# jrl-umi3218/lexls

Measured on AMD Instinct MI355X. Metric: batched fp64 l-QR factorizations/s (factorize+solve), higher is better.
Workload: dtype f64

## Files before the change

lexls_amd/csrc/lqr_qtol_body.inc:

```
            static_assert(NS >= 1 && NS <= 4 && MD <= 16 && (MD % 4) == 0, "shape limits of the row layout / two row parts of even size");
            constexpr int NH  = 2;
            constexpr int RP  = MD / NH;
            constexpr int HP  = RP / 2;
            constexpr int kHandoffStride = 8 * MD + 16;
            constexpr int NIH = NS * HP;
#ifndef LEXLS_QTOL_PF_STEPS
#define LEXLS_QTOL_PF_STEPS 9
#endif
            constexpr int PF_STEPS = LEXLS_QTOL_PF_STEPS < MD ? LEXLS_QTOL_PF_STEPS : MD;
            extern __shared__ double smem[];
            typedef __attribute__((address_space(3))) char lds_char;
            const int lds0 = (int)(unsigned)(size_t)(lds_char *)smem;
            const int lane = threadIdx.x & 63;
            const uint32_t wq = QT_WPB > 1 ? blockIdx.x * QT_WPB + (uint32_t)__builtin_amdgcn_readfirstlane((int)(threadIdx.x >> 6)) : blockIdx.x;
            if (wq * 4u >= a.batch) return;
            if constexpr (EST)
            {
                if (wq == 0 && lane == 0) *count_reset = 0u;
            }
            const int g    = lane >> 4;
            const int gl   = lane & 15;
            const int n    = NV ? NV : (int)a.nVar;
            const int cap  = (int)a.cap;
            const int nObj = (int)a.nObj;
            const uint32_t b  = wq * 4u + (uint32_t)g;
            const uint32_t bb = b < a.batch ? b : a.batch - 1u;
            const bool live   = b < a.batch && !(a.skip && a.skip[bb]);
            const uint32_t pstride = (uint32_t)cap * (uint32_t)(n + 1);
            const double *inw      = a.in + (size_t)wq * 4u * pstride;
            const uint32_t poff    = (bb - wq * 4u) * pstride;
            uint32_t dpack = 0;
            int Frow       = 0;
            if constexpr (RAG)
            {
                static_assert(!EST && MD <= 15 && kQuadMaxObj <= 8, "four bits per level in one word; no estimating ragged form");
                const uint32_t dk = gl < nObj ? a.dims[(size_t)bb * (uint32_t)nObj + (uint32_t)gl] : 0u;
                const int dv      = (int)(dk < (uint32_t)MD ? dk : (uint32_t)MD);
                for_each_index<0, kQuadMaxObj>([&](auto kk) __attribute__((always_inline)) {
                    constexpr int k_ = decltype(kk)::value;
                    dpack |= (uint32_t)gbci<k_>(dv) << (4 * k_);
                });
            }
            auto rag_rows = [&](qt_d2 v, int R, int r, int d, double &lo, double &hi) __attribute__((always_inline)) {
                lo = sel(r < d, sel(R == cap - 1, v.y, v.x), 0.0);
                hi = sel(r + 1 < d, v.y, 0.0);
            };

            double blk0[NS][MD];
#pragma unroll
            for (int s = 0; s < NS; s++)
            {
                const int P       = 16 * s + gl - SIG;
                const int c       = (P >= 0 && P <= n) ? P : 0;
                if constexpr (RAG)
                {
                    const double *colp = inw + (poff + (uint32_t)(c * cap));
                    const int d0       = (int)(dpack & 15u);
#pragma unroll
                    for (int r = 0; r < MD / 2; r++)
                    {
                        const int Rc  = 2 * r < cap - 2 ? 2 * r : cap - 2;
                        const qt_d2 v = *reinterpret_cast<const qt_d2u *>(colp + Rc);
                        rag_rows(v, 2 * r, 2 * r, d0, blk0[s][2 * r], blk0[s][2 * r + 1]);
                    }
                }
                else
                {
                    const qt_d2 *src2 = reinterpret_cast<const qt_d2 *>(inw + (poff + (uint32_t)(c * cap)));
#pragma unroll
                    for (int r = 0; r < MD / 2; r++)
                    {
                        const qt_d2 v      = src2[r];
                        blk0[s][2 * r]     = v.x;
                        blk0[s][2 * r + 1] = v.y;
                    }
                }
            }

            const int o_img   = lds0 + (int)((QT_WPB > 1 ? (threadIdx.x >> 6) * 4u : 0u) + (uint32_t)g) * (int)group_bytes;
            const int o_xs    = o_img + 8 * (int)img_doubles;
            const int o_ex    = o_xs + 8 * 16 * NS;
            const int o_phys  = o_ex + 8 * MD;
            const int o_perm  = o_phys + 64;
            const int o_meta  = o_perm + 64;
            const int o_emap  = o_meta + 16 * kQuadMaxObj;
            const int o_stage = o_emap + 8 * 16 * NS;
            auto D   = [&](int off) -> __attribute__((address_space(3))) double & { return *(__attribute__((address_space(3))) double *)(size_t)(unsigned)off; };
            auto D2  = [&](int off) -> __attribute__((address_space(3))) qt_d2 & { return *(__attribute__((address_space(3))) qt_d2 *)(size_t)(unsigned)off; };
            auto B8  = [&](int off) -> __attribute__((address_space(3))) uint8_t & { return *(__attribute__((address_space(3))) uint8_t *)(size_t)(unsigned)off; };
            auto U32 = [&](int off) -> __attribute__((address_space(3))) uint32_t & { return *(__attribute__((address_space(3))) uint32_t *)(size_t)(unsigned)off; };
            auto U64 = [&](int off) -> __attribute__((address_space(3))) unsigned long long & { return *(__attribute__((address_space(3))) unsigned long long *)(size_t)(unsigned)off; };
            typedef unsigned qt_u4 __attribute__((ext_vector_type(4)));
            auto U4 = [&](int off) -> __attribute__((address_space(3))) qt_u4 & { return *(__attribute__((address_space(3))) qt_u4 *)(size_t)(unsigned)off; };

#pragma unroll
            for (int s = 0; s < 4; s++) B8(o_phys + 16 * s + gl) = (uint8_t)(16 * s + gl);
#pragma unroll
            for (int s = 0; s < NS; s++)
            {
                D(o_emap + 8 * (16 * s + gl)) = 0.0;
                D(o_xs + 8 * (16 * s + gl))   = 0.0;
            }
            quad_lds_fence();

            if (stagger)
            {
                const unsigned simd = __builtin_amdgcn_s_getreg((4 << 0) | (4 << 6) | ((2 - 1) << 11));
                for (unsigned i = 0; i < simd * stagger; i++) __builtin_amdgcn_s_sleep(8);
            }

            const int CH = (n + 1) * HP;
            static_assert(NH * NIH <= 18, "eighteen piece registers");
            uint32_t pieceoff[NH * NIH];
            for_each_index<0, NH * NIH>([&](auto tt) __attribute__((always_inline)) {
                constexpr int t = decltype(tt)::value, h = t / NIH, i = t % NIH;
                int ch        = 16 * i + gl;
                ch            = ch < CH ? ch : CH - 1;
                const int col = ch / HP, m = ch - col * HP;
                if constexpr (RAG)
                    pieceoff[t] = ((uint32_t)(col * cap) << 2) | (uint32_t)m;
                else
                    pieceoff[t] = 8u * (poff + (uint32_t)(col * cap + h * RP + 2 * m));
            });
            static_assert(HP <= 4, "two bits for the pair index of a ragged piece");
            auto prefetch_piece = [&](auto tt, int Flev) __attribute__((always_inline)) {
                constexpr int t = decltype(tt)::value, i = t % NIH;
                if (16 * i < CH)
                {
                    if constexpr (RAG)
                    {
                        constexpr int h = t / NIH;
                        const int R     = Flev + h * RP + 2 * (int)(pieceoff[t] & 3u);
                        qt_pf_load<t>(inw, 8u * (poff + (pieceoff[t] >> 2) + (uint32_t)(R < cap - 2 ? R : cap - 2)));
                    }
                    else
                        qt_pf_load<t>(inw + Flev, pieceoff[t]);
                }
            };

            int rp[NS];
            int rq[NS];
            unsigned long long em[NS];
            int pos[NS];
            int pc[NS];
#pragma unroll
            for (int s = 0; s < NS; s++)
            {
                rp[s]  = o_xs;
                rq[s]  = 0x0c0c0c00;
                em[s]  = 0ull;
                pos[s] = 0;
                pc[s]  = 0;
            }

            int ColIndex   = 0;
            int TotalRank  = 0;
            int imgoff     = 0;
            bool exh       = false;
            bool have_next = false;
            double est2    = 0.0;
            double rsq[NS];
            STAMP_DECL
            STAMP(0)
#ifdef LEXLS_QTOL_CHAIN
            unsigned long long cacc[7] = {0, 0, 0, 0, 0, 0, 0};
#endif
#ifdef LEXLS_WAVE_STAMPS
            unsigned long long lst_t0 = clock64();
#endif

            constexpr bool PEEL = !(EST && NS == 3 && MD == 12);
            struct qt_level
            {
                bool work;
                int F;
                int dlev;
                int Fc;
                int rank;
                bool prefetch;
            };

            auto level_head = [&](auto l0c, const int k, qt_level &L) __attribute__((always_inline)) {
                constexpr bool L0 = decltype(l0c)::value;
                QT_LMARK("level-top")
                L.work = live && !exh;
                L.F    = RAG ? Frow : k * MD;
                L.dlev = RAG ? (int)((dpack >> (4 * k)) & 15u) : MD;
                if constexpr (RAG) Frow += L.dlev;
                L.Fc   = ColIndex;
                L.rank = 0;
                if (__ballot(L.work) == 0ull)
                {
                    if (gl == 0)
                    {
                        U32(o_meta + 16 * k)      = (uint32_t)L.Fc;
                        U32(o_meta + 16 * k + 4)  = 0u;
                        U32(o_meta + 16 * k + 8)  = (uint32_t)imgoff;
                        U32(o_meta + 16 * k + 12) = (uint32_t)(n + 1 - L.Fc);
                    }
                    return false;
                }
                if constexpr (!L0)
                {
                    if ((PEEL || k > 0) && !have_next)
                        for_each_index<0, NH * NIH>([&](auto tt) __attribute__((always_inline)) { prefetch_piece(tt, L.F); });
                }
                return true;
            };

            auto level_start = [&](const int k, const qt_level &L, double (&blk)[NS][MD]) __attribute__((always_inline)) {
                const int F = L.F, dlev = L.dlev;
                (void)F, (void)dlev;
                QT_MARK("level-start")
#pragma unroll
                for (int s = 0; s < NS; s++)
                {
                    const int P  = 16 * s + gl - SIG;
                    const int ph = (int)B8(o_phys + (P >= 0 && P < n ? P : 0));
                    pc[s]        = (P >= 0 && P < n) ? ph : (P == n ? n : 0);
                    pos[s]       = (P >= 0 && P <= n) ? P : 0x3fffff;
                }
#pragma unroll
                for (int s = 0; s < NS; s++) em[s] = U64(o_emap + 8 * pc[s]);
                if (PEEL || k > 0)
                for_each_index<0, NH>([&](auto hh) __attribute__((always_inline)) {
                    constexpr int h = decltype(hh)::value;
                    QT_MARK1("level-stage", h)
                    if constexpr (h == 0) asm volatile("s_waitcnt vmcnt(0)" ::: "memory");
                    for_each_index<0, NIH>([&](auto ii) __attribute__((always_inline)) {
                        constexpr int i = decltype(ii)::value;
                        if (16 * i < CH)
                        {
                            int ch = 16 * i + gl;
                            ch     = ch < CH ? ch : CH - 1;
                            qt_pf_store_lds<h * NIH + i>(o_stage + 16 * ch);
                        }
                    });
                    quad_lds_fence();
#pragma unroll
                    for (int s = 0; s < NS; s++)
                    {
#pragma unroll
                        for (int m = 0; m < HP; m++)
                        {
                            const qt_d2 v            = D2(o_stage + 16 * (pc[s] * HP + m));
                            if constexpr (RAG)
                                rag_rows(v, F + h * RP + 2 * m, h * RP + 2 * m, dlev, blk[s][h * RP + 2 * m], blk[s][h * RP + 2 * m + 1]);
                            else
                            {
                                blk[s][h * RP + 2 * m]     = v.x;
                                blk[s][h * RP + 2 * m + 1] = v.y;
                            }
                        }
                    }
                    quad_lds_fence();
                });
            };

            auto level_post = [&](auto l0c, const int k, qt_level &L, double (&blk)[NS][MD]) __attribute__((always_inline)) {
                constexpr bool L0 = decltype(l0c)::value;
                const bool work = L.work;
                const int Fc    = L.Fc;
                (void)k;
                STAMP(1)
                LSTAMP(0)
                QT_LMARK("level-post")
                if constexpr (EST)
                {
#pragma unroll
                    for (int s = 0; s < NS; s++)
                    {
                        double t = 0.0;
#pragma unroll
                        for (int r = 0; r < MD; r++) t = dfma(blk[s][r], blk[s][r], t);
                        rsq[s] = t;
                    }
                }
                L.prefetch = (k + 1 < nObj) && (rows_min(work ? Fc : 0x3fffffff) + MD < n);
                have_next  = L.prefetch;
            };

            auto eliminate = [&](const int k, const qt_level &L, double (&blk)[NS][MD]) __attribute__((always_inline)) {
                (void)k;
                const int Fcmax = rows_max(L.work ? L.Fc : 0);
                {
                    auto fetch_u = [&](auto cc, double (&u)[NS]) __attribute__((always_inline)) {
                        constexpr int C  = decltype(cc)::value;
                        constexpr int sc = (C + SIG) / 16, lc = (C + SIG) % 16;
                        const int rowp   = gbci<lc>(rp[sc]);
                        const int selq   = gbci<lc>(rq[sc]);
#pragma unroll
                        for (int s = sc; s < NS; s++)
                        {
                            const unsigned e = __builtin_amdgcn_perm((unsigned)(em[s] >> 32), (unsigned)em[s], (unsigned)selq);
                            u[s]             = D(rowp + (int)(e << 3));
                        }
                    };
                    double ua[NS], ub[NS];
#pragma unroll
                    for (int s = 0; s < NS; s++) ua[s] = ub[s] = 0.0;
                    if (Fcmax > 0) fetch_u(std::integral_constant<int, 0>{}, ua);
                    qt_for_each_while<0, 16 * NS - SIG>(
                        [&](auto cc) __attribute__((always_inline)) { return decltype(cc)::value < Fcmax; },
                        [&](auto cc) __attribute__((always_inline)) {
                            constexpr int C  = decltype(cc)::value;
                            constexpr int sc = (C + SIG) / 16, lc = (C + SIG) % 16;
                            double(&ucur)[NS]  = (C & 1) ? ub : ua;
                            double(&unext)[NS] = (C & 1) ? ua : ub;
                            QT_MARK1("elim", C)
                            if constexpr (NS - sc <= 2)
                            {
                                if constexpr (sc + 1 < NS) qt_gauss_dpp<lc>(blk[sc + 1], blk[sc], ucur[sc + 1]);
                                if constexpr (C + 1 < 16 * NS - SIG)
                                {
                                    if (C + 1 < Fcmax) fetch_u(std::integral_constant<int, C + 1>{}, unext);
                                }
                                qt_gauss_dpp_self<lc>(blk[sc], ucur[sc]);
                            }
                            else
                            {
                                double lr[MD];
                                for_each_index<0, MD>([&](auto rr) {
                                    constexpr int r = decltype(rr)::value;
                                    lr[r]           = gbc<lc>(blk[sc][r]);
                                });
#pragma unroll
                                for (int r = 0; r < MD; r++) blk[sc][r] = dfma(-lr[r], ucur[sc], blk[sc][r]);
                                if constexpr (C + 1 < 16 * NS - SIG)
                                {
                                    if (C + 1 < Fcmax) fetch_u(std::integral_constant<int, C + 1>{}, unext);
                                }
#pragma unroll
                                for (int s = sc + 1; s < NS; s++)
                                {
#pragma unroll
                                    for (int r = 0; r < MD; r++) blk[s][r] = dfma(-lr[r], ucur[s], blk[s][r]);
                                }
                            }
                        });
                    asm volatile("s_nop 1");
                }
                STAMP(7)
                LSTAMP(1)
            };

                auto factor_level = [&](auto l0c, auto s0c, qt_level &L, double (&blk)[NS][MD]) __attribute__((always_inline)) {
                    constexpr bool L0 = decltype(l0c)::value;
                    constexpr int S0 = decltype(s0c)::value;
                    constexpr int SL = NS - S0;
                    static_assert(!L0 || S0 == 0, "level 0 starts at column 0: every slot is live");
                    const bool work = L.work, prefetch = L.prefetch;
                    const int F = L.F, dlev = L.dlev;
                    int &rank = L.rank;
                    QT_LMARK1("hh-pro", S0)
                    double nrm[NS];
#pragma unroll
                    for (int s = S0; s < NS; s++)
                    {
                        double t = 0.0;
#pragma unroll
                        for (int r = 0; r < MD; r++) t = dfma(blk[s][r], blk[s][r], t);
                        nrm[s] = sel(pos[s] >= ColIndex && pos[s] < n, t, qt_with_hi(t, kQtSentinelHi));
                    }
                    bool go = work;
#ifdef LEXLS_QTOL_CHAIN
                    unsigned long long ct[7] = {0, 0, 0, 0, 0, 0, 0}, cp1 = 0;
                    bool cvalid = false;
#endif
                    int cur_lbs = S0, nxt_lbs = S0;
                    bool cur_ispl = false, nxt_ispl = false;
                    unsigned cur_w = 0, nxt_w = 0;
                    double pbest = 0.0;
                    auto decide_local = [&]() __attribute__((always_inline)) {
#pragma unroll
                        for (int s = S0; s < NS; s++)
                        {
                            const int kinv  = (0xFFF - ((s << 4) | gl)) - (pos[s] << 6);
                            const double pv = __hiloint2double(__double2hiint(nrm[s]), (__double2loint(nrm[s]) & ~0xFFF) | kinv);
                            pbest           = s == S0 ? pv : vmax(pbest, pv);
                        }
                        nxt_lbs = ((0xFFF - (__double2loint(pbest) & 0xFFF)) >> 4) & 3;
                    };
                    auto decide_finish = [&](double m) __attribute__((always_inline)) {
                        const int mlo = __double2loint(m);
                        nxt_w         = (unsigned)(0xFFF - (mlo & 0xFFF));
                        nxt_ispl      = ((__double2loint(pbest) ^ mlo) & 0xFFF) == 0;
                    };
                    {
                        decide_local();
                        decide_finish(row_max16(pbest));
                        double colv[MD];
#pragma unroll
                        for (int r = 0; r < MD; r++) colv[r] = blk[S0][r];
#pragma unroll
                        for (int s = S0 + 1; s < NS; s++)
                        {
                            const bool pick = nxt_lbs == s;
#pragma unroll
                            for (int r = 0; r < MD; r++) colv[r] = sel(pick, blk[s][r], colv[r]);
                        }
#pragma unroll
                        for (int r = 0; r < MD; r += 2) D2(o_stage + gl * kHandoffStride + 8 * r) = qt_d2{colv[r], colv[r + 1]};
                        cur_lbs = nxt_lbs, cur_ispl = nxt_ispl, cur_w = nxt_w;
                    }
                    double coln[MD];
                    auto fetch_column = [&](auto jjc, unsigned w) __attribute__((always_inline)) {
                        constexpr int ce0 = decltype(jjc)::value & ~1;
                        quad_lds_fence();
                        const int src = o_stage + (int)(w & 15u) * kHandoffStride;
#pragma unroll
                        for (int r = ce0; r < MD; r += 2)
                        {
                            const qt_d2 v   = D2(src + 8 * r);
                            coln[r]         = v.x;
                            coln[r + 1]     = v.y;
                        }
                    };
                    fetch_column(std::integral_constant<int, 0>{}, cur_w);

                    int pf_issued = 0;
                    qt_for_each_while<0, MD>(
                        [&](auto jc) __attribute__((always_inline)) { return (decltype(jc)::value % 4 != 0) || __ballot(go) != 0ull; },
                        [&](auto cnt) __attribute__((always_inline)) {
                        constexpr int j   = decltype(cnt)::value;
                        constexpr int ce  = j & ~1;
                        constexpr int cen = (j + 1) & ~1;
                        QT_LMARK2("hh-step", S0, j)
                        {
                            constexpr int TOT = NH * NIH, PF_PER = (TOT + PF_STEPS - 1) / PF_STEPS;
                            constexpr int lo = (j * PF_PER < TOT ? j * PF_PER : TOT), hi = ((j + 1) * PF_PER < TOT ? (j + 1) * PF_PER : TOT);
                            if (prefetch) for_each_index<lo, hi>([&](auto tt) __attribute__((always_inline)) { prefetch_piece(tt, F + dlev); });
                            pf_issued = hi;
                        }
                        const bool act = go;
                        CSTAMP(0, (int)cur_w)
                        double col[MD];
#pragma unroll
                        for (int r = ce; r < MD; r++) col[r] = coln[r];
                        FSTAMP(2)
                        CSTAMP(1, __double2loint(col[MD - 1]))
                        CSTAMP_COLLECT
                        const double c0 = col[j];
                        double t0 = 0.0, t1 = 0.0, t2 = 0.0;
#pragma unroll
                        for (int r = j + 1; r < MD; r++)
                        {
                            if ((r - j) % 3 == 1) t0 = dfma(col[r], col[r], t0);
                            if ((r - j) % 3 == 2) t1 = dfma(col[r], col[r], t1);
                            if ((r - j) % 3 == 0) t2 = dfma(col[r], col[r], t2);
                        }
                        const double tailSq = (t0 + t1) + t2;
                        const double fresh  = dfma(c0, c0, tailSq);
                        CSTAMP(2, __double2loint(fresh))
                        const bool cont     = RAG ? (act && !(fresh < a.tol) && j < dlev) : (act && !(fresh < a.tol));
                        go                  = cont;
                        double g, h;
                        {
                            const double y = __builtin_amdgcn_rsq(fresh);
                            g              = fresh * y;
                            h              = 0.5 * y;
                            double r       = dfma(-h, g, 0.5);
                            g              = dfma(g, r, g);
                            h              = dfma(h, r, h);
#ifndef LEXLS_QTOL_ONE_NEWTON
                            r              = dfma(-h, g, 0.5);
                            g              = dfma(g, r, g);
                            h              = dfma(h, r, h);
#endif
                        }
                        const bool neg    = c0 >= 0.0;
                        const double beta = neg ? -g : g;
                        const double ibet = (neg ? -2.0 : 2.0) * h;
                        CSTAMP(3, __double2loint(ibet))
                        const double rden = qt_rcp1(c0 - beta);
                        double dw[NS];
#pragma unroll
                        for (int s = S0; s < NS; s++)
                        {
                            double d0 = 0.0, d1 = 0.0;
#pragma unroll
                            for (int r = j + 1; r < MD; r++)
                            {
                                if ((r - j) & 1)
                                    d0 = dfma(col[r], blk[s][r], d0);
                                else
                                    d1 = dfma(col[r], blk[s][r], d1);
                            }
                            dw[s] = dfma(c0, blk[s][j], d0 + d1);
                        }
                        FSTAMP(3)
                        double gs[NS];
#pragma unroll
                        for (int s = S0; s < NS; s++)
                        {
                            const double t = dw[s] * ibet;
                            gs[s]          = (t - blk[s][j]) * rden;
                            nrm[s]         = dfma(-t, t, nrm[s]);
                            nrm[s]         = sel(cont && cur_ispl && cur_lbs == s, qt_with_hi(nrm[s], kQtSentinelHi), nrm[s]);
                            blk[s][j]      = t * ibet;
                        }
                        CSTAMP(4, __double2hiint(nrm[NS - 1]))
                        const int ppos = (int)(cur_w >> 6);
#pragma unroll
                        for (int s = S0; s < NS; s++)
                        {
                            const bool front = cont && pos[s] == ColIndex;
                            pos[s]           = sel(front, ppos, pos[s]);
                            pos[s]           = sel(cont && cur_ispl && cur_lbs == s, ColIndex, pos[s]);
                        }
                        B8(sel(cont && cur_ispl, o_perm + ColIndex, o_ex + 4 * gl)) = (uint8_t)ppos;
                        if constexpr (EST)
                        {
                            double r2 = rsq[S0];
#pragma unroll
                            for (int s = S0 + 1; s < NS; s++) r2 = sel(cur_lbs == s, rsq[s], r2);
                            est2 = sel(cont && cur_ispl, vmax(est2, r2 * (h * h)), est2);
                        }
                        ColIndex += cont ? 1 : 0;
                        rank += cont ? 1 : 0;
                        const bool full = cont && ColIndex == n;
                        exh             = exh || full;
                        go              = go && !full;
                        FSTAMP(4)
                        if constexpr (j + 1 < MD && SL == 1)
                        {
                            decide_local();
                            double m = pbest;
                            auto upd_rows = [&](auto qq) __attribute__((always_inline)) {
                                constexpr int q = decltype(qq)::value;
#pragma unroll
                                for (int r = j + 1; r < MD; r++)
                                    if ((r - j - 1) % 4 == q) blk[S0][r] = dfma(gs[S0], col[r], blk[S0][r]);
                            };
                            m = dpp_max<0xB1>(m);
                            upd_rows(std::integral_constant<int, 0>{});
                            m = dpp_max<0x4E>(m);
                            upd_rows(std::integral_constant<int, 1>{});
                            m = dpp_max<0x141>(m);
                            upd_rows(std::integral_constant<int, 2>{});
                            m = dpp_max<0x140>(m);
                            upd_rows(std::integral_constant<int, 3>{});
#pragma unroll
                            for (int r = cen; r < MD; r += 2) D2(o_stage + gl * kHandoffStride + 8 * r) = qt_d2{blk[S0][r], blk[S0][r + 1]};
                            decide_finish(m);
                            fetch_column(std::integral_constant<int, j + 1>{}, nxt_w);
                        }
                        else if constexpr (j + 1 < MD)
                        {
                            decide_local();
                            double colv[MD];
                            double gsb = gs[S0];
                            double m   = pbest;
                            auto pick_rows = [&](auto qq) __attribute__((always_inline)) {
                                constexpr int q = decltype(qq)::value;
#pragma unroll
                                for (int r = cen; r < MD; r++)
                                    if ((r - cen) % 4 == q)
                                    {
                                        colv[r] = blk[S0][r];
#pragma unroll
                                        for (int s = S0 + 1; s < NS; s++) colv[r] = sel(nxt_lbs == s, blk[s][r], colv[r]);
                                    }
                            };
                            m = dpp_max<0xB1>(m);
                            pick_rows(std::integral_constant<int, 0>{});
                            m = dpp_max<0x4E>(m);
                            pick_rows(std::integral_constant<int, 1>{});
                            m = dpp_max<0x141>(m);
                            pick_rows(std::integral_constant<int, 2>{});
                            m = dpp_max<0x140>(m);
                            pick_rows(std::integral_constant<int, 3>{});
#pragma unroll
                            for (int s = S0 + 1; s < NS; s++) gsb = sel(nxt_lbs == s, gs[s], gsb);
#pragma unroll
                            for (int r = (cen > j + 1 ? cen : j + 1); r < MD; r++) colv[r] = dfma(gsb, col[r], colv[r]);
#pragma unroll
                            for (int r = cen; r < MD; r += 2) D2(o_stage + gl * kHandoffStride + 8 * r) = qt_d2{colv[r], colv[r + 1]};
                            decide_finish(m);
                            fetch_column(std::integral_constant<int, j + 1>{}, nxt_w);
                        }
                        CSTAMP(5, (int)nxt_w)
                        if constexpr (!(j + 1 < MD && SL == 1))
                        {
#pragma unroll
                            for (int s = S0; s < NS; s++)
                            {
#pragma unroll
                                for (int r = j + 1; r < MD; r++) blk[s][r] = dfma(gs[s], col[r], blk[s][r]);
                            }
                        }
                        cur_lbs = nxt_lbs, cur_ispl = nxt_ispl, cur_w = nxt_w;
                        CSTAMP(6, __double2loint(blk[NS - 1][MD - 1]))
                        FSTAMP(5)
                    });
                    QT_LMARK1("hh-end", S0)
                    if (prefetch)
                        for_each_index<0, NH * NIH>([&](auto tt) __attribute__((always_inline)) {
                            if (decltype(tt)::value >= pf_issued) prefetch_piece(tt, F + dlev);
                        });
                    (void)SL;
                };

            auto level_end = [&](auto l0c, const int k, const qt_level &L, double (&blk)[NS][MD]) __attribute__((always_inline)) {
                constexpr bool L0 = decltype(l0c)::value;
                const bool work = L.work;
                const int Fc = L.Fc, rank = L.rank;
                STAMP(5)
                LSTAMP(2)
                QT_LMARK("level-end")
                const int wk   = n + 1 - Fc;
                const int dump = o_stage + 8 * gl;
                int roff[MD];
#pragma unroll
                for (int p = 0; p < MD; p++) roff[p] = 8 * (p * wk - p * (p + 1) / 2);
#pragma unroll
                for (int s = 0; s < NS; s++)
                {
                    const int P0  = 16 * s + gl - SIG;
                    const bool mv = work && P0 <= n && P0 >= Fc;
                    const int e   = pos[s] - Fc;
                    const int lim = mv ? (e < rank - 1 ? e : rank - 1) : -1;
                    const int base = o_img + 8 * (imgoff + e);
                    if (mv)
                    {
                        QT_LMARK1("level-end-store", s)
#pragma unroll
                        for (int p = 0; p < MD; p++) D(sel(p <= lim, base + roff[p], dump)) = blk[s][p];
                        B8(o_emap + 8 * pc[s] + k) = (uint8_t)e;
                        if (P0 < n) B8(o_phys + pos[s]) = (uint8_t)pc[s];
                    }
                    QT_LMARK1("level-end-maps", s)
                    const bool piv = work && P0 >= Fc && P0 < Fc + rank;
                    const int p    = P0 - Fc;
                    rp[s]          = sel(piv, o_img + 8 * (imgoff + p * wk - p * (p + 1) / 2), rp[s]);
                    rq[s]          = sel(piv, 0x0c0c0c00 | k, rq[s]);
                }
                STAMP(6)
                LSTAMP(3)
                if (gl == 0)
                {
                    U32(o_meta + 16 * k)      = (uint32_t)Fc;
                    U32(o_meta + 16 * k + 4)  = (uint32_t)rank;
                    U32(o_meta + 16 * k + 8)  = (uint32_t)imgoff;
                    U32(o_meta + 16 * k + 12) = (uint32_t)wk;
                }
                quad_lds_fence();
                imgoff += wk * rank - rank * (rank - 1) / 2;
                TotalRank += rank;
            };

            if constexpr (PEEL)
            {
                qt_level L;
                if (level_head(std::true_type{}, 0, L))
                {
#pragma unroll
                    for (int s = 0; s < NS; s++)
                    {
                        const int P = 16 * s + gl - SIG;
                        pc[s]       = (P >= 0 && P <= n) ? P : 0;
                        pos[s]      = (P >= 0 && P <= n) ? P : 0x3fffff;
                        em[s]       = 0ull;
                    }
                    level_post(std::true_type{}, 0, L, blk0);
                    {
                        constexpr int k = 0;
                        (void)k;
                        STAMP(7)
                        LSTAMP(1)
                    }
                    factor_level(std::true_type{}, std::integral_constant<int, 0>{}, L, blk0);
                    level_end(std::true_type{}, 0, L, blk0);
                }
            }

            for (int k = PEEL ? 1 : 0; k < nObj; k++)
            {
                qt_level L;
                if (!level_head(std::false_type{}, k, L)) continue;
                double blk_k[NS][MD];
                double(&blk)[NS][MD] = *(PEEL ? &blk_k : &blk0);
                level_start(k, L, blk);
                level_post(std::false_type{}, k, L, blk);
                eliminate(k, L, blk);
                QT_MARK("hh-select")
                {
                    const int s0 = (rows_min(L.work ? L.Fc : 0x3fffffff) + SIG) >> 4;
                    if (NS > 3 && s0 >= 3)
                        factor_level(std::false_type{}, std::integral_constant<int, (NS > 3 ? 3 : 0)>{}, L, blk);
                    else if (NS > 2 && s0 >= 2)
                        factor_level(std::false_type{}, std::integral_constant<int, (NS > 2 ? 2 : 0)>{}, L, blk);
                    else if (NS > 1 && s0 >= 1)
                        factor_level(std::false_type{}, std::integral_constant<int, (NS > 1 ? 1 : 0)>{}, L, blk);
                    else
                        factor_level(std::false_type{}, std::integral_constant<int, 0>{}, L, blk);
                }
                level_end(std::false_type{}, k, L, blk);
            }

            QT_MARK("solve-top")
            const int o_zero = o_xs + 8 * (16 * NS - 1);
            for (int k = nObj; k--;)
            {
                QT_MARK("solve-level")
                const qt_u4 mt = U4(o_meta + 16 * k);
                const int rank = live ? (int)mt.y : 0;
                const int rmax = rows_max(rank);
                if (rmax == 0) continue;
                const int Fc = (int)mt.x, ok = (int)mt.z, wk = (int)mt.w;
                const int c0   = Fc + rank;
                const int acc  = rank > 0 ? TotalRank - c0 : 0;
                const int amax = rows_max(acc);
                const int p    = gl < rank ? gl : 0;
                const int row  = o_img + 8 * (ok + p * wk - p * (p + 1) / 2);
                double col[MD];
#pragma unroll
                for (int j = 1; j < MD; j++) col[j] = D(sel(j < rank && gl < j, row + 8 * j, o_zero));
                double sv = D(sel(gl < rank, row + 8 * (n - Fc), o_zero));
                for (int base = 0; base < amax; base += 16)
                {
                    QT_MARK("solve-trip")
                    const bool have = base + gl < acc;
                    const int c     = have ? c0 + base + gl : 16 * NS - 1;
                    const int ph    = (int)B8(o_phys + c);
                    const int offv  = have ? (int)B8(o_emap + 8 * ph + k) : 0;
                    const double xv = D(o_xs + 8 * c);
                    double uj[16];
                    for_each_index<0, 16>([&](auto jj) {
                        constexpr int j = decltype(jj)::value;
                        uj[j]           = D(row + 8 * gbci<j>(offv));
                    });
                    __builtin_amdgcn_sched_barrier(0);
                    double s0 = 0.0, s1 = 0.0;
                    for_each_index<0, 16>([&](auto jj) {
                        constexpr int j = decltype(jj)::value;
                        if (j & 1)
                            s1 = dfma(-uj[j], gbc<j>(xv), s1);
                        else
                            s0 = dfma(-uj[j], gbc<j>(xv), s0);
                    });
                    sv += s0 + s1;
                }
                QT_MARK("solve-tail")
                sv = sel(gl < rank, sv, 0.0);
                for_each_index<1, MD>([&](auto jj) {
                    constexpr int j = MD - decltype(jj)::value;
                    sv = dfma(-col[j], gbc<j>(sv), sv);
                });
                D(sel(gl < rank, o_xs + 8 * (Fc + gl), o_stage + 8 * gl)) = sv;
                quad_lds_fence();
            }
            STAMP(9)
            QT_MARK("output")
            if (live)
            {
#pragma unroll
                for (int s = 0; s < NS; s++)
                {
                    const int P = 16 * s + gl;
                    if (P < n)
                    {
                        a.x[(size_t)b * n + B8(o_phys + P)] = D(o_xs + 8 * P);
                        a.perm[(size_t)b * n + P]           = (P < TotalRank) ? (uint32_t)B8(o_perm + P) : (uint32_t)P;
                    }
                }
                if (gl < nObj)
                {
                    a.fcol[(size_t)b * nObj + gl] = U32(o_meta + 16 * gl);
                    a.rank[(size_t)b * nObj + gl] = U32(o_meta + 16 * gl + 4);
                }
                if (gl == 0) a.totalrank[b] = (uint32_t)TotalRank;
            }
            if constexpr (EST)
            {
                const double e2 = row_max16(est2);
                if (gl == 0 && live) est_out[b] = e2 > 0.0 ? 2.0 * qt_sqrt(e2) : 0.0;
            }
            STAMP(10)
            STAMP_WRITE
#ifdef LEXLS_QTOL_CHAIN
            if (lane == 0)
                for (int i_ = 0; i_ < 7; i_++) a.lambda[(size_t)b * (n + cap) + 30 + i_] = (double)cacc[i_];
#endif
```

lexls_amd/csrc/lqr_qtol_impl.h:

```cpp
#pragma once
#include "lqr_quad_impl.h"

#include <cstdlib>


namespace lexls
{
    namespace
    {
        __device__ __forceinline__ double qt_rcp(double x)
        {
            double y = __builtin_amdgcn_rcp(x);
            double e = dfma(-x, y, 1.0);
            y        = dfma(y, e, y);
            e        = dfma(-x, y, 1.0);
            return dfma(y, e, y);
        }

        __device__ __forceinline__ double qt_rcp1(double x)
        {
            const double y = __builtin_amdgcn_rcp(x);
            return dfma(y, dfma(-x, y, 1.0), y);
        }

        __device__ __forceinline__ double qt_sqrt(double x)
        {
            const double y = __builtin_amdgcn_rsq(x);
            double g       = x * y;
            double h       = 0.5 * y;
            const double r = dfma(-h, g, 0.5);
            g              = dfma(g, r, g);
            h              = dfma(h, r, h);
            double d       = dfma(-g, g, x);
            g              = dfma(d, h, g);
            d              = dfma(-g, g, x);
            return dfma(d, h, g);
        }

        __device__ __forceinline__ double qt_with_hi(double v, int hi) { return __hiloint2double(hi, __double2loint(v)); }

#ifdef LEXLS_WAVE_STAMPS_FINE
#define FSTAMP(i) if constexpr (S0 == LEXLS_WAVE_STAMPS_FINE) STAMP(i)
#else
#define FSTAMP(i)
#endif
#ifdef LEXLS_QTOL_CHAIN
#define CSTAMP(i, val)                                                                                     \
    if constexpr (S0 == LEXLS_QTOL_CHAIN)                                                                  \
    {                                                                                                      \
        int dummy_;                                                                                        \
        asm volatile("v_mov_b32 %1, %2\n\ts_memtime %0" : "=s"(ct[i]), "=v"(dummy_) : "v"(val));         \
    }
#define CSTAMP_COLLECT                                                                                     \
    if constexpr (S0 == LEXLS_QTOL_CHAIN)                                                                  \
    {                                                                                                      \
        asm volatile("s_waitcnt lgkmcnt(0)" ::: "memory");                                                 \
        if (cvalid)                                                                                        \
        {                                                                                                  \
            cacc[2] += ct[2] - cp1; cacc[3] += ct[3] - ct[2]; cacc[4] += ct[4] - ct[3];                     \
            cacc[5] += ct[5] - ct[4]; cacc[6] += ct[6] - ct[5]; cacc[0] += ct[0] - ct[6];                   \
        }                                                                                                  \
        cacc[1] += ct[1] - ct[0];                                                                          \
        cp1    = ct[1];                                                                                    \
        cvalid = true;                                                                                     \
    }
#else
#define CSTAMP(i, val)
#define CSTAMP_COLLECT
#endif
#ifdef LEXLS_WAVE_STAMPS
#define LSTAMP(ph)                                                                                   \
    {                                                                                                \
        const unsigned long long t_ = clock64();                                                     \
        if (gl == 0 && live) a.lambda[(size_t)b * (n + cap) + 11 + 4 * k + (ph)] = (double)(t_ - lst_t0); \
        lst_t0 = t_;                                                                                 \
    }
#else
#define LSTAMP(ph)
#endif
#ifdef LEXLS_QTOL_MARKS
#define QT_MARK(name) asm volatile("; qtol-region " name);
#define QT_MARK1(name, i) asm volatile("; qtol-region " name " %0" ::"i"(i));
#define QT_MARK2(name, i, j) asm volatile("; qtol-region " name " %0 %1" ::"n"(i), "n"(j));
#else
#define QT_MARK(name)
#define QT_MARK1(name, i)
#define QT_MARK2(name, i, j)
#endif
#define QT_LMARK(name)        if constexpr (L0) { QT_MARK("level0-" name) } else { QT_MARK(name) }
#define QT_LMARK1(name, i)    if constexpr (L0) { QT_MARK1("level0-" name, i) } else { QT_MARK1(name, i) }
#define QT_LMARK2(name, i, j) if constexpr (L0) { QT_MARK2("level0-" name, i, j) } else { QT_MARK2(name, i, j) }
        template <int B, int E, class P, class F>
        __device__ __forceinline__ void qt_for_each_while(P &&pred, F &&f)
        {
            if constexpr (B < E)
            {
                if (pred(std::integral_constant<int, B>{}))
                {
                    f(std::integral_constant<int, B>{});
                    qt_for_each_while<B + 1, E>(pred, f);
                }
            }
        }

        typedef double qt_d2 __attribute__((ext_vector_type(2)));
        typedef qt_d2 qt_d2u __attribute__((aligned(8)));


#define QT_PF_LIST(X) X(0, 184, 187) X(1, 188, 191) X(2, 192, 195) X(3, 196, 199) X(4, 200, 203) X(5, 204, 207) X(6, 208, 211) X(7, 212, 215) X(8, 216, 219) \
    X(9, 220, 223) X(10, 224, 227) X(11, 228, 231) X(12, 232, 235) X(13, 236, 239) X(14, 240, 243) X(15, 244, 247) X(16, 248, 251) X(17, 252, 255)
        template <int T>
        __device__ __forceinline__ void qt_pf_load(const double *base, uint32_t byte_offset)
        {
#define QT_PF_LOAD(t, lo, hi) \
    if constexpr (T == t) asm volatile("global_load_dwordx4 a[" #lo ":" #hi "], %0, %1" ::"v"(byte_offset), "s"(base) : "memory", "a" #lo, "a" #hi);
            QT_PF_LIST(QT_PF_LOAD)
#undef QT_PF_LOAD
        }
        template <int T>
        __device__ __forceinline__ void qt_pf_store_lds(int lds_byte_address)
        {
#define QT_PF_STORE(t, lo, hi) \
    if constexpr (T == t) asm volatile("ds_write_b128 %0, a[" #lo ":" #hi "]" ::"v"(lds_byte_address) : "memory");
            QT_PF_LIST(QT_PF_STORE)
#undef QT_PF_STORE
        }

#define QT_FD(i) "v_fmac_f64_dpp %[d" #i "], %[s" #i "], -%[u] row_newbcast:%[l] row_mask:0xf bank_mask:0xf\n\t"
#define QT_FS(i) "v_fmac_f64_dpp %[d" #i "], %[d" #i "], -%[u] row_newbcast:%[l] row_mask:0xf bank_mask:0xf\n\t"
#define QT_FO(i) [d##i] "+v"(d[i])
#define QT_FI(i) [s##i] "v"(s[i])
        template <int L, int MD>
        __device__ __forceinline__ void qt_gauss_dpp(double (&d)[MD], const double (&s)[MD], double u)
        {
            static_assert(MD == 8 || MD == 12, "operand lists below");
            if constexpr (MD == 8)
                asm volatile("s_nop 1\n\t" QT_FD(0) QT_FD(1) QT_FD(2) QT_FD(3) QT_FD(4) QT_FD(5) QT_FD(6) QT_FD(7)
                             : QT_FO(0), QT_FO(1), QT_FO(2), QT_FO(3), QT_FO(4), QT_FO(5), QT_FO(6), QT_FO(7)
                             : QT_FI(0), QT_FI(1), QT_FI(2), QT_FI(3), QT_FI(4), QT_FI(5), QT_FI(6), QT_FI(7), [u] "v"(u), [l] "n"(L));
            else
                asm volatile("s_nop 1\n\t" QT_FD(0) QT_FD(1) QT_FD(2) QT_FD(3) QT_FD(4) QT_FD(5) QT_FD(6) QT_FD(7) QT_FD(8) QT_FD(9) QT_FD(10) QT_FD(11)
                             : QT_FO(0), QT_FO(1), QT_FO(2), QT_FO(3), QT_FO(4), QT_FO(5), QT_FO(6), QT_FO(7), QT_FO(8), QT_FO(9), QT_FO(10), QT_FO(11)
                             : QT_FI(0), QT_FI(1), QT_FI(2), QT_FI(3), QT_FI(4), QT_FI(5), QT_FI(6), QT_FI(7), QT_FI(8), QT_FI(9), QT_FI(10), QT_FI(11),
                               [u] "v"(u), [l] "n"(L));
        }
        template <int L, int MD>
        __device__ __forceinline__ void qt_gauss_dpp_self(double (&d)[MD], double u)
        {
            static_assert(MD == 8 || MD == 12, "operand lists below");
            if constexpr (MD == 8)
                asm volatile("s_nop 1\n\t" QT_FS(0) QT_FS(1) QT_FS(2) QT_FS(3) QT_FS(4) QT_FS(5) QT_FS(6) QT_FS(7)
                             : QT_FO(0), QT_FO(1), QT_FO(2), QT_FO(3), QT_FO(4), QT_FO(5), QT_FO(6), QT_FO(7)
                             : [u] "v"(u), [l] "n"(L));
            else
                asm volatile("s_nop 1\n\t" QT_FS(0) QT_FS(1) QT_FS(2) QT_FS(3) QT_FS(4) QT_FS(5) QT_FS(6) QT_FS(7) QT_FS(8) QT_FS(9) QT_FS(10) QT_FS(11)
                             : QT_FO(0), QT_FO(1), QT_FO(2), QT_FO(3), QT_FO(4), QT_FO(5), QT_FO(6), QT_FO(7), QT_FO(8), QT_FO(9), QT_FO(10), QT_FO(11)
                             : [u] "v"(u), [l] "n"(L));
        }
#undef QT_FD
#undef QT_FS
#undef QT_FO
#undef QT_FI

        constexpr int kQtSentinelHi = (int)0xFFE00000;

        template <int NS, int MD, int SIG, int NV>
        __global__ __launch_bounds__(64 * QT_WPB) void lqr_qtol_kernel(LseArgs a, uint32_t img_doubles, uint32_t group_bytes, uint32_t stagger)
        {
            constexpr bool EST           = false;
            constexpr bool RAG           = false;
            double *const est_out        = nullptr;
            uint32_t *const count_reset  = nullptr;
#include "lqr_qtol_body.inc"
        }

        template <int NS, int MD, int SIG, int NV>
        __global__ __launch_bounds__(64 * QT_WPB) void lqr_qtol_rag_kernel(LseArgs a, uint32_t img_doubles, uint32_t group_bytes, uint32_t stagger)
        {
            constexpr bool EST           = false;
            constexpr bool RAG           = true;
            double *const est_out        = nullptr;
            uint32_t *const count_reset  = nullptr;
#include "lqr_qtol_body.inc"
        }

        template <int NS, int MD, int SIG, int NV>
        __global__ __launch_bounds__(64 * QT_WPB) void lqr_qtol_est_kernel(LseArgs a, uint32_t img_doubles, uint32_t group_bytes, uint32_t stagger, double *est_out,
                                                                          uint32_t *count_reset)
        {
            constexpr bool EST = true;
            constexpr bool RAG = false;
            if constexpr (NS == 3 && MD == 12 && NV == 0)
            {
#include "lqr_qtol_body_unpeeled.inc"
            }
            else
            {
#include "lqr_qtol_body.inc"
            }
        }

        template <int NS, int MD, int SIG, int NV, bool EST = false, bool RAG = false>
        hipError_t launch_qtol_t(const LseArgs &a, hipStream_t s, double *est_out = nullptr, uint32_t *count_reset = nullptr)
        {
            static_assert(!(EST && RAG), "no estimating ragged form");
            const void *kfn;
            if constexpr (RAG)
                kfn = reinterpret_cast<const void *>(lqr_qtol_rag_kernel<NS, MD, SIG, NV>);
            else if constexpr (EST)
                kfn = reinterpret_cast<const void *>(lqr_qtol_est_kernel<NS, MD, SIG, NV>);
            else
                kfn = reinterpret_cast<const void *>(lqr_qtol_kernel<NS, MD, SIG, NV>);
            const uint32_t img  = qtol_image_doubles(a.nVar, a.nObj, MD);
            const size_t gbytes = qtol_group_bytes<NS, MD>(a.nVar, a.nObj);
            const size_t lds    = qtol_lds_bytes<NS, MD>(a.nVar, a.nObj);
            if (lds > kMaxLdsBytes || a.nObj > (uint32_t)kQuadMaxObj || a.nVar + 1 + SIG > 16u * NS || a.nVar > 63u || (NV && a.nVar != (uint32_t)NV)) return hipErrorInvalidValue;
            if ((reinterpret_cast<uintptr_t>(a.in) & (RAG ? 7u : 15u)) || a.nfixed || a.reg_type != 0) return hipErrorInvalidValue;
            if (RAG ? (a.cap < 2u || !a.dims) : (a.uniform_dim != (uint32_t)MD || (a.cap & 1u))) return hipErrorInvalidValue;
            if (lds > 64 * 1024)
            {
                static size_t granted[64] = {0};
                int dev = 0;
                if (hipGetDevice(&dev) != hipSuccess || dev < 0 || dev >= 64) dev = -1;
                if (dev < 0 || granted[dev] < lds)
                {
                    hipError_t e = hipFuncSetAttribute(kfn, hipFuncAttributeMaxDynamicSharedMemorySize, (int)lds);
                    if (e != hipSuccess) return e;
                    if (dev >= 0) granted[dev] = lds;
                }
            }
            const uint32_t blocks = (a.batch + 4u * QT_WPB - 1u) / (4u * QT_WPB);
            static const uint32_t stagger = std::getenv("LEXLS_QTOL_STAGGER") ? (uint32_t)std::atoi(std::getenv("LEXLS_QTOL_STAGGER")) : 0u;
            if constexpr (RAG)
                hipLaunchKernelGGL((lqr_qtol_rag_kernel<NS, MD, SIG, NV>), dim3(blocks), dim3(64 * QT_WPB), lds, s, a, img, (uint32_t)gbytes, stagger);
            else if constexpr (EST)
                hipLaunchKernelGGL((lqr_qtol_est_kernel<NS, MD, SIG, NV>), dim3(blocks), dim3(64 * QT_WPB), lds, s, a, img, (uint32_t)gbytes, stagger, est_out, count_reset);
            else
                hipLaunchKernelGGL((lqr_qtol_kernel<NS, MD, SIG, NV>), dim3(blocks), dim3(64 * QT_WPB), lds, s, a, img, (uint32_t)gbytes, stagger);
            return hipGetLastError();
        }
    }
}

#define LEXLS_QTOL_INSTANCE(NAME, NS, MD, SIG, NV) \
    namespace lexls { hipError_t NAME(const LseArgs &a, hipStream_t s) { return launch_qtol_t<NS, MD, SIG, NV>(a, s); } }
#define LEXLS_QTOL_INSTANCE_EST(NAME, NS, MD, SIG, NV) \
    namespace lexls { hipError_t NAME(const LseArgs &a, hipStream_t s, double *est_out, uint32_t *count_reset) { return launch_qtol_t<NS, MD, SIG, NV, true>(a, s, est_out, count_reset); } }
#define LEXLS_QTOL_INSTANCE_RAG(NAME, NS, MD, SIG, NV) \
    namespace lexls { hipError_t NAME(const LseArgs &a, hipStream_t s) { return launch_qtol_t<NS, MD, SIG, NV, false, true>(a, s); } }
```

Measured before the change: 103.7 million.

## Retire the lone leading column slot after step zero in the factor level

Adds a specialised factor_level form used when every row's level starts on the last column of slot NS-2. After Householder step 0 that slot's remaining column is written out to the image and moved into the last slot through LDS. Later steps then loop over one fewer slot, cutting the FMA, norm and select work. The cost is an extra LDS exchange and fence, a larger code footprint and more register pressure. The path only runs for compile-time shapes where qt_retire_reachable holds and the runtime uniformity test passes.

```diff
diff --git a/lexls_amd/csrc/lqr_qtol_body.inc b/lexls_amd/csrc/lqr_qtol_body.inc
--- a/lexls_amd/csrc/lqr_qtol_body.inc
+++ b/lexls_amd/csrc/lqr_qtol_body.inc
@@ -170,6 +170,8 @@
 #endif
 
             constexpr bool PEEL = !(EST && NS == 3 && MD == 12);
+            constexpr int kRetireSlot = NS - 2;
+            constexpr bool RETIRE     = !EST && !RAG && PEEL && NV > 0 && qt_retire_reachable(NS, MD, SIG, NV) && 8 * (NV + 1) * RP >= 17 * kHandoffStride;
             struct qt_level
             {
                 bool work;
@@ -344,15 +346,18 @@
                 LSTAMP(1)
             };
 
-                auto factor_level = [&](auto l0c, auto s0c, qt_level &L, double (&blk)[NS][MD]) __attribute__((always_inline)) {
+                auto factor_level = [&](auto l0c, auto s0c, auto retc, const int k, qt_level &L, double (&blk)[NS][MD]) __attribute__((always_inline)) {
                     constexpr bool L0 = decltype(l0c)::value;
                     constexpr int S0 = decltype(s0c)::value;
+                    constexpr bool RET = decltype(retc)::value;
                     constexpr int SL = NS - S0;
                     static_assert(!L0 || S0 == 0, "level 0 starts at column 0: every slot is live");
+                    static_assert(!RET || (RETIRE && !L0 && S0 == kRetireSlot && SL == 2), "the retiring form: two live slots, one behind step 0");
+                    (void)k;
                     const bool work = L.work, prefetch = L.prefetch;
                     const int F = L.F, dlev = L.dlev;
                     int &rank = L.rank;
-                    QT_LMARK1("hh-pro", S0)
+                    if constexpr (RET) { QT_MARK1("hh-ret-pro", S0) } else { QT_LMARK1("hh-pro", S0) }
                     double nrm[NS];
 #pragma unroll
                     for (int s = S0; s < NS; s++)
@@ -371,13 +376,14 @@
                     bool cur_ispl = false, nxt_ispl = false;
                     unsigned cur_w = 0, nxt_w = 0;
                     double pbest = 0.0;
-                    auto decide_local = [&]() __attribute__((always_inline)) {
-#pragma unroll
-                        for (int s = S0; s < NS; s++)
+                    auto decide_local = [&](auto loc) __attribute__((always_inline)) {
+                        constexpr int LO = decltype(loc)::value;
+#pragma unroll
+                        for (int s = LO; s < NS; s++)
                         {
                             const int kinv  = (0xFFF - ((s << 4) | gl)) - (pos[s] << 6);
                             const double pv = __hiloint2double(__double2hiint(nrm[s]), (__double2loint(nrm[s]) & ~0xFFF) | kinv);
-                            pbest           = s == S0 ? pv : vmax(pbest, pv);
+                            pbest           = s == LO ? pv : vmax(pbest, pv);
                         }
                         nxt_lbs = ((0xFFF - (__double2loint(pbest) & 0xFFF)) >> 4) & 3;
                     };
@@ -387,7 +393,7 @@
                         nxt_ispl      = ((__double2loint(pbest) ^ mlo) & 0xFFF) == 0;
                     };
                     {
-                        decide_local();
+                        decide_local(std::integral_constant<int, S0>{});
                         decide_finish(row_max16(pbest));
                         double colv[MD];
 #pragma unroll
@@ -425,7 +431,12 @@
                         constexpr int j   = decltype(cnt)::value;
                         constexpr int ce  = j & ~1;
                         constexpr int cen = (j + 1) & ~1;
-                        QT_LMARK2("hh-step", S0, j)
+                        constexpr int SJ  = (RET && j >= 1) ? S0 + 1 : S0;
+                        constexpr int SLJ = NS - SJ;
+                        if constexpr (RET) { QT_MARK2("hh-ret-step", S0, j) } else { QT_LMARK2("hh-step", S0, j) }
+                        const unsigned w0 = cur_w;
+                        const bool ispl0  = cur_ispl;
+                        (void)w0, (void)ispl0;
                         {
                             constexpr int TOT = NH * NIH, PF_PER = (TOT + PF_STEPS - 1) / PF_STEPS;
                             constexpr int lo = (j * PF_PER < TOT ? j * PF_PER : TOT), hi = ((j + 1) * PF_PER < TOT ? (j + 1) * PF_PER : TOT);
@@ -475,7 +486,7 @@
                         const double rden = qt_rcp1(c0 - beta);
                         double dw[NS];
 #pragma unroll
-                        for (int s = S0; s < NS; s++)
+                        for (int s = SJ; s < NS; s++)
                         {
                             double d0 = 0.0, d1 = 0.0;
 #pragma unroll
@@ -491,7 +502,7 @@
                         FSTAMP(3)
                         double gs[NS];
 #pragma unroll
-                        for (int s = S0; s < NS; s++)
+                        for (int s = SJ; s < NS; s++)
                         {
                             const double t = dw[s] * ibet;
                             gs[s]          = (t - blk[s][j]) * rden;
@@ -502,7 +513,7 @@
                         CSTAMP(4, __double2hiint(nrm[NS - 1]))
                         const int ppos = (int)(cur_w >> 6);
 #pragma unroll
-                        for (int s = S0; s < NS; s++)
+                        for (int s = SJ; s < NS; s++)
                         {
                             const bool front = cont && pos[s] == ColIndex;
                             pos[s]           = sel(front, ppos, pos[s]);
@@ -511,9 +522,9 @@
                         B8(sel(cont && cur_ispl, o_perm + ColIndex, o_ex + 4 * gl)) = (uint8_t)ppos;
                         if constexpr (EST)
                         {
-                            double r2 = rsq[S0];
-#pragma unroll
-                            for (int s = S0 + 1; s < NS; s++) r2 = sel(cur_lbs == s, rsq[s], r2);
+                            double r2 = rsq[SJ];
+#pragma unroll
+                            for (int s = SJ + 1; s < NS; s++) r2 = sel(cur_lbs == s, rsq[s], r2);
                             est2 = sel(cont && cur_ispl, vmax(est2, r2 * (h * h)), est2);
                         }
                         ColIndex += cont ? 1 : 0;
@@ -522,15 +533,15 @@
                         exh             = exh || full;
                         go              = go && !full;
                         FSTAMP(4)
-                        if constexpr (j + 1 < MD && SL == 1)
-                        {
-                            decide_local();
+                        if constexpr (j + 1 < MD && SLJ == 1)
+                        {
+                            decide_local(std::integral_constant<int, SJ>{});
                             double m = pbest;
                             auto upd_rows = [&](auto qq) __attribute__((always_inline)) {
                                 constexpr int q = decltype(qq)::value;
 #pragma unroll
                                 for (int r = j + 1; r < MD; r++)
-                                    if ((r - j - 1) % 4 == q) blk[S0][r] = dfma(gs[S0], col[r], blk[S0][r]);
+                                    if ((r - j - 1) % 4 == q) blk[SJ][r] = dfma(gs[SJ], col[r], blk[SJ][r]);
                             };
                             m = dpp_max<0xB1>(m);
                             upd_rows(std::integral_constant<int, 0>{});
@@ -541,15 +552,15 @@
                             m = dpp_max<0x140>(m);
                             upd_rows(std::integral_constant<int, 3>{});
 #pragma unroll
-                            for (int r = cen; r < MD; r += 2) D2(o_stage + gl * kHandoffStride + 8 * r) = qt_d2{blk[S0][r], blk[S0][r + 1]};
+                            for (int r = cen; r < MD; r += 2) D2(o_stage + gl * kHandoffStride + 8 * r) = qt_d2{blk[SJ][r], blk[SJ][r + 1]};
                             decide_finish(m);
                             fetch_column(std::integral_constant<int, j + 1>{}, nxt_w);
                         }
                         else if constexpr (j + 1 < MD)
                         {
-                            decide_local();
+                            decide_local(std::integral_constant<int, SJ>{});
                             double colv[MD];
-                            double gsb = gs[S0];
+                            double gsb = gs[SJ];
                             double m   = pbest;
                             auto pick_rows = [&](auto qq) __attribute__((always_inline)) {
                                 constexpr int q = decltype(qq)::value;
@@ -557,9 +568,9 @@
                                 for (int r = cen; r < MD; r++)
                                     if ((r - cen) % 4 == q)
                                     {
-                                        colv[r] = blk[S0][r];
-#pragma unroll
-                                        for (int s = S0 + 1; s < NS; s++) colv[r] = sel(nxt_lbs == s, blk[s][r], colv[r]);
+                                        colv[r] = blk[SJ][r];
+#pragma unroll
+                                        for (int s = SJ + 1; s < NS; s++) colv[r] = sel(nxt_lbs == s, blk[s][r], colv[r]);
                                     }
                             };
                             m = dpp_max<0xB1>(m);
@@ -571,7 +582,7 @@
                             m = dpp_max<0x140>(m);
                             pick_rows(std::integral_constant<int, 3>{});
 #pragma unroll
-                            for (int s = S0 + 1; s < NS; s++) gsb = sel(nxt_lbs == s, gs[s], gsb);
+                            for (int s = SJ + 1; s < NS; s++) gsb = sel(nxt_lbs == s, gs[s], gsb);
 #pragma unroll
                             for (int r = (cen > j + 1 ? cen : j + 1); r < MD; r++) colv[r] = dfma(gsb, col[r], colv[r]);
 #pragma unroll
@@ -580,20 +591,74 @@
                             fetch_column(std::integral_constant<int, j + 1>{}, nxt_w);
                         }
                         CSTAMP(5, (int)nxt_w)
-                        if constexpr (!(j + 1 < MD && SL == 1))
-                        {
-#pragma unroll
-                            for (int s = S0; s < NS; s++)
+                        if constexpr (!(j + 1 < MD && SLJ == 1))
+                        {
+#pragma unroll
+                            for (int s = SJ; s < NS; s++)
                             {
 #pragma unroll
                                 for (int r = j + 1; r < MD; r++) blk[s][r] = dfma(gs[s], col[r], blk[s][r]);
                             }
                         }
                         cur_lbs = nxt_lbs, cur_ispl = nxt_ispl, cur_w = nxt_w;
+                        if constexpr (RET && j == 0)
+                        {
+                            QT_MARK1("hh-retire", S0)
+                            const int x0  = (int)(w0 & 15u);
+                            const int ws0 = (int)((w0 >> 4) & 3u);
+                            {
+                                double w00 = blk[S0][0];
+                                int wpc    = pc[S0];
+#pragma unroll
+                                for (int s = S0 + 1; s < NS; s++)
+                                {
+                                    w00 = sel(ws0 == s, blk[s][0], w00);
+                                    wpc = sel(ws0 == s, pc[s], wpc);
+                                }
+                                if (cont && ispl0)
+                                {
+                                    D(o_img + 8 * imgoff)     = w00;
+                                    B8(o_emap + 8 * wpc + k)  = (uint8_t)0;
+                                    B8(o_phys + L.Fc)         = (uint8_t)wpc;
+                                }
+                            }
+                            const int o_mv  = o_stage + 16 * kHandoffStride;
+                            const bool mrow = cont && ws0 != S0;
+                            if (mrow && gl == 15)
+                            {
+#pragma unroll
+                                for (int r = 0; r < MD; r += 2) D2(o_mv + 8 * r) = qt_d2{blk[S0][r], blk[S0][r + 1]};
+                                D2(o_mv + 8 * MD) = qt_d2{nrm[S0], __hiloint2double(pc[S0], pos[S0])};
+                            }
+                            quad_lds_fence();
+                            double mc[MD];
+#pragma unroll
+                            for (int r = 0; r < MD; r += 2)
+                            {
+                                const qt_d2 v = D2(o_mv + 8 * r);
+                                mc[r]         = v.x;
+                                mc[r + 1]     = v.y;
+                            }
+                            const qt_d2 mt  = D2(o_mv + 8 * MD);
+                            const bool recv = mrow && gl == x0;
+#pragma unroll
+                            for (int s = S0 + 1; s < NS; s++)
+                            {
+                                const bool hit = SL == 2 ? recv : (recv && ws0 == s);
+#pragma unroll
+                                for (int r = 0; r < MD; r++) blk[s][r] = sel(hit, mc[r], blk[s][r]);
+                                nrm[s] = sel(hit, mt.x, nrm[s]);
+                                pos[s] = sel(hit, __double2loint(mt.y), pos[s]);
+                                pc[s]  = sel(hit, __double2hiint(mt.y), pc[s]);
+                            }
+                            const bool lone1 = mrow && (int)((cur_w >> 4) & 3u) == S0;
+                            cur_ispl         = lone1 ? gl == x0 : cur_ispl;
+                            cur_lbs          = lone1 ? ws0 : cur_lbs;
+                        }
                         CSTAMP(6, __double2loint(blk[NS - 1][MD - 1]))
                         FSTAMP(5)
                     });
-                    QT_LMARK1("hh-end", S0)
+                    if constexpr (RET) { QT_MARK1("hh-ret-end", S0) } else { QT_LMARK1("hh-end", S0) }
                     if (prefetch)
                         for_each_index<0, NH * NIH>([&](auto tt) __attribute__((always_inline)) {
                             if (decltype(tt)::value >= pf_issued) prefetch_piece(tt, F + dlev);
@@ -601,8 +666,9 @@
                     (void)SL;
                 };
 
-            auto level_end = [&](auto l0c, const int k, const qt_level &L, double (&blk)[NS][MD]) __attribute__((always_inline)) {
+            auto level_end = [&](auto l0c, const int k, const qt_level &L, double (&blk)[NS][MD], const bool retired) __attribute__((always_inline)) {
                 constexpr bool L0 = decltype(l0c)::value;
+                (void)retired;
                 const bool work = L.work;
                 const int Fc = L.Fc, rank = L.rank;
                 STAMP(5)
@@ -617,7 +683,11 @@
                 for (int s = 0; s < NS; s++)
                 {
                     const int P0  = 16 * s + gl - SIG;
-                    const bool mv = work && P0 <= n && P0 >= Fc;
+                    bool mv       = work && P0 <= n && P0 >= Fc;
+                    if constexpr (RETIRE && !L0)
+                    {
+                        if (s == kRetireSlot) mv = mv && !(retired && rank > 0);
+                    }
                     const int e   = pos[s] - Fc;
                     const int lim = mv ? (e < rank - 1 ? e : rank - 1) : -1;
                     const int base = o_img + 8 * (imgoff + e);
@@ -669,8 +739,8 @@
                         STAMP(7)
                         LSTAMP(1)
                     }
-                    factor_level(std::true_type{}, std::integral_constant<int, 0>{}, L, blk0);
-                    level_end(std::true_type{}, 0, L, blk0);
+                    factor_level(std::true_type{}, std::integral_constant<int, 0>{}, std::false_type{}, 0, L, blk0);
+                    level_end(std::true_type{}, 0, L, blk0, false);
                 }
             }
 
@@ -684,18 +754,24 @@
                 level_post(std::false_type{}, k, L, blk);
                 eliminate(k, L, blk);
                 QT_MARK("hh-select")
-                {
-                    const int s0 = (rows_min(L.work ? L.Fc : 0x3fffffff) + SIG) >> 4;
-                    if (NS > 3 && s0 >= 3)
-                        factor_level(std::false_type{}, std::integral_constant<int, (NS > 3 ? 3 : 0)>{}, L, blk);
+                bool retired = false;
+                {
+                    const int fcmin = rows_min(L.work ? L.Fc : 0x3fffffff);
+                    const int s0    = (fcmin + SIG) >> 4;
+                    if constexpr (RETIRE)
+                        retired = __ballot(!L.work) == 0ull && rows_max(L.Fc) == fcmin && s0 == kRetireSlot && ((fcmin + SIG) & 15) == 15;
+                    if (RETIRE && retired)
+                        factor_level(std::false_type{}, std::integral_constant<int, (RETIRE ? kRetireSlot : 0)>{}, std::integral_constant<bool, RETIRE>{}, k, L, blk);
+                    else if (NS > 3 && s0 >= 3)
+                        factor_level(std::false_type{}, std::integral_constant<int, (NS > 3 ? 3 : 0)>{}, std::false_type{}, k, L, blk);
                     else if (NS > 2 && s0 >= 2)
-                        factor_level(std::false_type{}, std::integral_constant<int, (NS > 2 ? 2 : 0)>{}, L, blk);
+                        factor_level(std::false_type{}, std::integral_constant<int, (NS > 2 ? 2 : 0)>{}, std::false_type{}, k, L, blk);
                     else if (NS > 1 && s0 >= 1)
-                        factor_level(std::false_type{}, std::integral_constant<int, (NS > 1 ? 1 : 0)>{}, L, blk);
+                        factor_level(std::false_type{}, std::integral_constant<int, (NS > 1 ? 1 : 0)>{}, std::false_type{}, k, L, blk);
                     else
-                        factor_level(std::false_type{}, std::integral_constant<int, 0>{}, L, blk);
-                }
-                level_end(std::false_type{}, k, L, blk);
+                        factor_level(std::false_type{}, std::integral_constant<int, 0>{}, std::false_type{}, k, L, blk);
+                }
+                level_end(std::false_type{}, k, L, blk, retired);
             }
 
             QT_MARK("solve-top")
diff --git a/lexls_amd/csrc/lqr_qtol_impl.h b/lexls_amd/csrc/lqr_qtol_impl.h
--- a/lexls_amd/csrc/lqr_qtol_impl.h
+++ b/lexls_amd/csrc/lqr_qtol_impl.h
@@ -164,6 +164,16 @@
 
         constexpr int kQtSentinelHi = (int)0xFFE00000;
 
+        constexpr bool qt_retire_reachable(int NS, int MD, int SIG, int NV)
+        {
+            for (int k = 1; k < kQuadMaxObj; k++)
+            {
+                const int fc = k * MD;
+                if (fc < NV && ((fc + SIG) & 15) == 15 && ((fc + SIG) >> 4) == NS - 2) return true;
+            }
+            return false;
+        }
+
         template <int NS, int MD, int SIG, int NV>
         __global__ __launch_bounds__(64 * QT_WPB) void lqr_qtol_kernel(LseArgs a, uint32_t img_doubles, uint32_t group_bytes, uint32_t stagger)
         {
```

Result: faster. 105.2 million (median of 6 runs) (+1.4%).
